# Chang-Tun-Yu/HLS-final-Visual-Odometry

Measured on AMD Instinct MI355X. Metric: stereo frame-pairs/sec (detect+match), KITTI 1241x376; matches bit-exact, higher is better.
Workload: dtype u8; 1 GPU; KITTI 1241x376 stereo quad-match (prev/curr x L/R), default 50x50 bins; noise=0, gpu_max_hw_queues=4, streams_per_gpu=256, frames_in_hbm=8, parallelism=1x independent stream groups

## Files before the change

hls-final-visual-odometry_amd/csrc/kernels_match.hip:

```cpp
#include "vh_dev.h"
#include <algorithm>
#include <cstdlib>
#include <type_traits>

#ifdef VH_FLOW_STATS
__device__ unsigned long long g_flow_stats[12];
extern "C" int32_t vh_debug_flow_stats(unsigned long long *out, int32_t reset) {
  if (hipMemcpyFromSymbol(out, HIP_SYMBOL(g_flow_stats), sizeof(g_flow_stats)) != hipSuccess) return -3;
  if (reset) { unsigned long long z[12] = {0}; if (hipMemcpyToSymbol(HIP_SYMBOL(g_flow_stats), z, sizeof(z)) != hipSuccess) return -3; }
  return 0;
}
#define VH_STAT(k, n) do { if ((threadIdx.x & 63) == 0) atomicAdd(&g_flow_stats[k], (unsigned long long)(n)); } while (0)
#else
#define VH_STAT(k, n) do { } while (0)
#endif

#ifndef VH_MATCH_WAVES
#define VH_MATCH_WAVES 7
#endif
#ifndef VH_SNAKE
#define VH_SNAKE 1
#endif

namespace {

__device__ __forceinline__ int32_t indexed_count(const VhSets &s, int32_t set) { return s.bin_start[(int64_t)set * (s.nbins + 1) + s.nbins]; }

__device__ __forceinline__ int32_t wave_min(int32_t v) {
#pragma unroll
  for (int32_t d = 32; d >= 1; d >>= 1) v = min(v, __shfl_xor(v, d));
  return v;
}
__device__ __forceinline__ int32_t wave_max(int32_t v) {
#pragma unroll
  for (int32_t d = 32; d >= 1; d >>= 1) v = max(v, __shfl_xor(v, d));
  return v;
}

typedef unsigned short us2 __attribute__((ext_vector_type(2)));
__device__ __forceinline__ us2 as_us2(uint32_t x) { return __builtin_bit_cast(us2, x); }
__device__ __forceinline__ uint32_t as_u32(us2 x) { return __builtin_bit_cast(uint32_t, x); }

__device__ __forceinline__ uint32_t sad4(uint32_t a, uint32_t b, uint32_t acc) {
  return __builtin_amdgcn_sad_u8(a, b, acc);
}
__device__ __forceinline__ uint32_t sad4hi(uint32_t a, uint32_t b, uint32_t acc) {
  return __builtin_amdgcn_sad_hi_u8(a, b, acc);
}

template <bool MAX>
__device__ __forceinline__ int32_t row16_allreduce(int32_t v) {
#define VH_ROW_STEP(CTRL)                                                                   \
  {                                                                                         \
    const int32_t t = __builtin_amdgcn_update_dpp(v, v, CTRL, 0xF, 0xF, false);             \
    v = MAX ? max(v, t) : min(v, t);                                                        \
  }
  VH_ROW_STEP(0x128)
  VH_ROW_STEP(0x124)
  VH_ROW_STEP(0x122)
  VH_ROW_STEP(0x121)
#undef VH_ROW_STEP
  return v;
}

template <bool TESTED, bool NEED_UV, class Consume>
__device__ __forceinline__ void walk_region(const VhSets &s, const int32_t *__restrict__ cbs, const uint32_t *__restrict__ cuv,
                                            const uint4 *__restrict__ cdesc, int32_t c, int32_t UB0, int32_t UB1, int32_t VB0,
                                            int32_t VB1, int32_t ULO_MAX, int32_t UHI_MIN, int32_t VA0, int32_t VA1,
                                            Consume consume) {
  const int32_t lane = threadIdx.x & 63;
  const bool merged = !TESTED && VB0 == 0 && VB1 == s.vbn - 1;
  const int32_t UB1w = merged ? UB0 : UB1;
  for (int32_t cb = UB0; cb <= UB1w; cb += 64) {
    const int32_t ncb = min(64, UB1w - cb + 1);
    int32_t t_p0 = 0, t_p1 = 0, t_a0 = 0, t_a1 = 0;
    if (lane < ncb) {
      const int32_t row = (c * s.ubn + cb + lane) * s.vbn;
      t_p0 = cbs[row + VB0]; t_p1 = merged ? cbs[(c * s.ubn + UB1 + 1) * s.vbn] : cbs[row + VB1 + 1];
      if (TESTED) {
        const int32_t ubx = cb + lane;
        const bool in_ = ubx * s.binsize >= ULO_MAX && ubx * s.binsize + s.binsize - 1 <= UHI_MIN;
        t_a0 = in_ ? ((VA0 <= VA1) ? cbs[row + VA0] : t_p1) : 1;
        t_a1 = in_ ? ((VA0 <= VA1) ? cbs[row + VA1 + 1] : t_p1) : 0;
      }
    }
    int32_t ci = -1, pc = -64, p1 = 0;
    const auto advance = [&]() -> bool {
      pc += 64;
      while (pc >= p1) {
        if (++ci >= ncb) return false;
        pc = __builtin_amdgcn_readlane(t_p0, ci); p1 = __builtin_amdgcn_readlane(t_p1, ci);
      }
      return true;
    };
    if (!advance()) continue;
    int32_t pl = min(pc + lane, p1 - 1);
    uint32_t gu = 0;
    if (NEED_UV) gu = cuv[pl];
    uint4 g0 = cdesc[2 * (int64_t)pl], g1 = cdesc[2 * (int64_t)pl + 1];
    for (;;) {
      const int32_t c_pc = pc, c_p1 = p1, c_ci = ci, c_pl = pl;
      const uint32_t c_gu = gu;
      const uint4 c_g0 = g0, c_g1 = g1;
      const bool more = advance();
      if (more) {
        pl = min(pc + lane, p1 - 1);
        if (NEED_UV) gu = cuv[pl];
        g0 = cdesc[2 * (int64_t)pl]; g1 = cdesc[2 * (int64_t)pl + 1];
      }
      int32_t pa0 = 1, pa1 = 0;
      if (TESTED) { pa0 = __builtin_amdgcn_readlane(t_a0, c_ci); pa1 = __builtin_amdgcn_readlane(t_a1, c_ci); }
      consume(c_pc, c_p1, pa0, pa1, c_pl, c_gu, c_g0, c_g1);
      if (!more) break;
    }
  }
}

__device__ __forceinline__ void glds16(const void *gsrc, uint32_t lds_dst) {
  asm volatile("s_mov_b32 m0, %1\n\ts_nop 0\n\tglobal_load_lds_dwordx4 %0, off" ::"v"(gsrc), "s"(lds_dst) : "memory");
}
__device__ __forceinline__ void glds4(const void *gsrc, uint32_t lds_dst) {
  asm volatile("s_mov_b32 m0, %1\n\ts_nop 0\n\tglobal_load_lds_dword %0, off" ::"v"(gsrc), "s"(lds_dst) : "memory");
}
__device__ __forceinline__ uint32_t lds_addr(const void *p) {
  return __builtin_amdgcn_readfirstlane((uint32_t)(uintptr_t)(const __attribute__((address_space(3))) void *)p);
}

template <bool TESTED, class Consume>
__device__ __forceinline__ void walk_region_lds(const VhSets &s, const int32_t *__restrict__ cbs, const uint32_t *__restrict__ cuv,
                                                const uint4 *__restrict__ cdesc, int32_t c, int32_t UB0, int32_t UB1, int32_t VB0,
                                                int32_t VB1, int32_t ULO_MAX, int32_t UHI_MIN, int32_t VA0, int32_t VA1,
                                                uint4 *wD, uint32_t *wU, Consume consume) {
  const int32_t lane = threadIdx.x & 63;
  const uint32_t ldsD = lds_addr(wD), ldsU = lds_addr(wU);
  const bool merged = !TESTED && VB0 == 0 && VB1 == s.vbn - 1;
  const int32_t UB1w = merged ? UB0 : UB1;
  for (int32_t cb = UB0; cb <= UB1w; cb += 64) {
    const int32_t ncb = min(64, UB1w - cb + 1);
    int32_t t_p0 = 0, t_p1 = 0, t_a0 = 0, t_a1 = 0;
    if (lane < ncb) {
      const int32_t row = (c * s.ubn + cb + lane) * s.vbn;
      t_p0 = cbs[row + VB0]; t_p1 = merged ? cbs[(c * s.ubn + UB1 + 1) * s.vbn] : cbs[row + VB1 + 1];
      if (TESTED) {
        const int32_t ubx = cb + lane;
        const bool in_ = ubx * s.binsize >= ULO_MAX && ubx * s.binsize + s.binsize - 1 <= UHI_MIN;
        t_a0 = in_ ? ((VA0 <= VA1) ? cbs[row + VA0] : t_p1) : 1;
        t_a1 = in_ ? ((VA0 <= VA1) ? cbs[row + VA1 + 1] : t_p1) : 0;
      }
    }
    int32_t ci = -1, pc = -64, p1 = 0;
    const auto advance = [&]() -> bool {
      pc += 64;
      while (pc >= p1) {
        if (++ci >= ncb) return false;
        pc = __builtin_amdgcn_readlane(t_p0, ci); p1 = __builtin_amdgcn_readlane(t_p1, ci);
      }
      return true;
    };
    const auto issue = [&](int32_t b) {
      const int32_t pl = min(pc + lane, p1 - 1);
      const uint4 *g = cdesc + 2 * (int64_t)pl;
      glds16(g, ldsD + (uint32_t)b * 2048u); glds16(g + 1, ldsD + (uint32_t)b * 2048u + 1024u);
      if (TESTED) glds4(cuv + pl, ldsU + (uint32_t)b * 256u);
    };
    if (!advance()) continue;
    asm volatile("s_waitcnt lgkmcnt(0)" ::: "memory");
    int32_t buf = 0;
    issue(0);
    for (;;) {
      const int32_t c_pc = pc, c_p1 = p1, c_ci = ci, c_buf = buf;
      const bool more = advance();
      if (more) {
        buf ^= 1;
        asm volatile("s_waitcnt lgkmcnt(0)" ::: "memory");
        issue(buf);
        if (TESTED) asm volatile("s_waitcnt vmcnt(3)" ::: "memory");
        else asm volatile("s_waitcnt vmcnt(2)" ::: "memory");
      } else {
        asm volatile("s_waitcnt vmcnt(0)" ::: "memory");
      }
      int32_t pa0 = 1, pa1 = 0;
      if (TESTED) { pa0 = __builtin_amdgcn_readlane(t_a0, c_ci); pa1 = __builtin_amdgcn_readlane(t_a1, c_ci); }
      consume(c_pc, c_p1, pa0, pa1, (const uint4 *)(wD + c_buf * 128), (const uint32_t *)(wU + c_buf * 64));
      if (!more) break;
    }
  }
}

__device__ __forceinline__ uint64_t tested_key_uniform_query(const uint32_t (&qd)[8], us2 lo2, us2 span2, uint32_t uv2,
                                                             const uint4 &b0, const uint4 &b1, uint32_t relpos) {
  const us2 t = as_us2(uv2) - lo2;
  const us2 m = __builtin_elementwise_min(t, span2);
  uint32_t sad = sad4(qd[0], b0.x, 0);
  sad = sad4(qd[1], b0.y, sad); sad = sad4(qd[2], b0.z, sad); sad = sad4(qd[3], b0.w, sad);
  sad = sad4(qd[4], b1.x, sad); sad = sad4(qd[5], b1.y, sad); sad = sad4(qd[6], b1.z, sad); sad = sad4(qd[7], b1.w, sad);
  return as_u32(t) != as_u32(m) ? ~0ull : (((uint64_t)sad << 32) | relpos);
}
__device__ __forceinline__ uint64_t shfl_xor_u64(uint64_t k, int32_t d) {
  const uint32_t lo = (uint32_t)__shfl_xor((int32_t)(uint32_t)k, d), hi = (uint32_t)__shfl_xor((int32_t)(uint32_t)(k >> 32), d);
  return ((uint64_t)hi << 32) | lo;
}
__device__ __forceinline__ uint64_t wave_min_u64(uint64_t k) {
#pragma unroll
  for (int32_t d = 32; d >= 1; d >>= 1) k = min(k, shfl_xor_u64(k, d));
  return k;
}

enum { KEY_HI16 = 0, KEY_W19 = 1, KEY_64 = 2 };
template <int KM> struct KeyT { typedef uint32_t type; };
template <> struct KeyT<KEY_64> { typedef uint64_t type; };
template <int KM>
__device__ __forceinline__ typename KeyT<KM>::type sad_key(const uint4 &a0, const uint4 &a1, const uint4 &b0, const uint4 &b1, uint32_t seed) {
  if (KM == KEY_HI16) {
    uint32_t key = sad4hi(a0.x, b0.x, seed);
    key = sad4hi(a0.y, b0.y, key); key = sad4hi(a0.z, b0.z, key); key = sad4hi(a0.w, b0.w, key);
    key = sad4hi(a1.x, b1.x, key); key = sad4hi(a1.y, b1.y, key); key = sad4hi(a1.z, b1.z, key); key = sad4hi(a1.w, b1.w, key);
    return (typename KeyT<KM>::type)key;
  }
  uint32_t sad = sad4(a0.x, b0.x, 0);
  sad = sad4(a0.y, b0.y, sad); sad = sad4(a0.z, b0.z, sad); sad = sad4(a0.w, b0.w, sad);
  sad = sad4(a1.x, b1.x, sad); sad = sad4(a1.y, b1.y, sad); sad = sad4(a1.z, b1.z, sad); sad = sad4(a1.w, b1.w, sad);
  if (KM == KEY_W19) return (typename KeyT<KM>::type)((sad << 19) | seed);
  return (typename KeyT<KM>::type)(((uint64_t)sad << 32) | seed);
}
template <int KM>
__device__ __forceinline__ uint64_t key_to_64(typename KeyT<KM>::type k) {
  if (KM == KEY_64) return (uint64_t)k;
  if ((uint32_t)k == 0xFFFFFFFFu) return ~0ull;
  const uint32_t kk = (uint32_t)k;
  return KM == KEY_HI16 ? (((uint64_t)(kk >> 16) << 32) | (kk & 0xFFFFu)) : (((uint64_t)(kk >> 19) << 32) | (kk & 0x7FFFFu));
}
__device__ __forceinline__ int32_t key_mode_of(int32_t class_count, int32_t wide_keys) {
  if (class_count + 64 <= 0x10000 && !wide_keys) return KEY_HI16;
  return class_count <= VH_CLASS_POS_MAX && wide_keys < 2 ? KEY_W19 : KEY_64;
}

#ifndef VH_REDO_G
#define VH_REDO_G 2
#endif
struct RedoGroup {
  uint32_t qd[VH_REDO_G][8];
  us2 lo2[VH_REDO_G];
  int32_t lane[VH_REDO_G], qi[VH_REDO_G], n;
  int32_t umin, umax, vmin, vmax;
};
template <int Q>
__device__ __forceinline__ bool redo_take(uint64_t (&todo)[Q], const uint4 (&a0)[Q], const uint4 (&a1)[Q], const uint32_t (&uv1)[Q],
                                          int32_t radius, int32_t rv, RedoGroup &g) {
  g.n = 0; g.umin = g.vmin = 0x7FFFFFFF; g.umax = g.vmax = -1;
#pragma unroll
  for (int32_t k = 0; k < VH_REDO_G; k++) {
    int32_t fl = -1, fq = 0;
#pragma unroll
    for (int32_t qi = 0; qi < Q; qi++)
      if (fl < 0 && todo[qi]) { fl = (int32_t)__builtin_ctzll(todo[qi]); fq = qi; todo[qi] &= todo[qi] - 1; }
    if (fl < 0) break;
    uint4 x0 = a0[0], x1 = a1[0];
    uint32_t xu = uv1[0];
#pragma unroll
    for (int32_t qi = 1; qi < Q; qi++) if (fq == qi) { x0 = a0[qi]; x1 = a1[qi]; xu = uv1[qi]; }
    g.qd[k][0] = __builtin_amdgcn_readlane(x0.x, fl); g.qd[k][1] = __builtin_amdgcn_readlane(x0.y, fl);
    g.qd[k][2] = __builtin_amdgcn_readlane(x0.z, fl); g.qd[k][3] = __builtin_amdgcn_readlane(x0.w, fl);
    g.qd[k][4] = __builtin_amdgcn_readlane(x1.x, fl); g.qd[k][5] = __builtin_amdgcn_readlane(x1.y, fl);
    g.qd[k][6] = __builtin_amdgcn_readlane(x1.z, fl); g.qd[k][7] = __builtin_amdgcn_readlane(x1.w, fl);
    const uint32_t quv1 = __builtin_amdgcn_readlane(xu, fl);
    const int32_t u1 = (int32_t)(quv1 & 0xFFFF), v1 = (int32_t)(quv1 >> 16);
    g.lo2[k] = us2{(unsigned short)(u1 - radius), (unsigned short)(v1 - rv)};
    g.lane[k] = fl; g.qi[k] = fq; g.n = k + 1;
    g.umin = min(g.umin, u1); g.umax = max(g.umax, u1); g.vmin = min(g.vmin, v1); g.vmax = max(g.vmax, v1);
  }
  return g.n > 0;
}

template <int Q> struct TileOut {
  uint64_t k[Q];
  uint4 a0[Q], a1[Q];
  uint32_t uv1[Q];
  int32_t qpos[Q];
  bool valid[Q];
};

template <int Q, int P, bool SPEC, bool FLOW>
__device__ __forceinline__ void finish_tile(const VhSets &s, const VhMatchArgs &a, int32_t pass, int32_t stream, int32_t qset, int32_t cset,
                                            int32_t c, int32_t pbase, int32_t pcnt, const TileOut<Q> &o,
                                            int32_t *__restrict__ best, int32_t *__restrict__ redo_count) {
  constexpr int L = 64 / P;
  const int32_t lane = threadIdx.x & 63, ph = lane / L;
  const uint32_t *__restrict__ cuv = s.s_uv + (int64_t)cset * s.cap;
  const uint4 *__restrict__ cdesc = (const uint4 *)(s.s_desc + (int64_t)cset * s.cap * 8);
  const int32_t *__restrict__ cbs = s.bin_start + (int64_t)cset * (s.nbins + 1);
  const int32_t rv = FLOW ? a.radius : a.disp_tol;
  const us2 span2 = {(unsigned short)(2 * a.radius), (unsigned short)(2 * rv)};
  const int32_t *__restrict__ cidx = s.s_idx + (int64_t)cset * s.cap;
  const int32_t *__restrict__ qidx = s.s_idx + (int64_t)qset * s.cap;
  int32_t *__restrict__ tbl = best + ((int64_t)stream * 4 + a.pass[pass].slot) * s.cap;
  int32_t res[Q];
  uint64_t todo[Q];
#pragma unroll
  for (int32_t qi = 0; qi < Q; qi++) {
    res[qi] = -1;
    bool fail = false;
    if (o.valid[qi] && ph == 0 && o.k[qi] != ~0ull) {
      int32_t wp = (int32_t)(uint32_t)o.k[qi];
      VH_CHECK_RANGE(s, 7, wp, 0, pcnt);
      res[qi] = pbase + wp;
      if (SPEC) {
        const int32_t u1 = o.uv1[qi] & 0xFFFF, v1 = o.uv1[qi] >> 16;
        const us2 lo2 = {(unsigned short)(u1 - a.radius), (unsigned short)(v1 - rv)};
        const us2 t = as_us2(cuv[res[qi]]) - lo2;
        const us2 m = __builtin_elementwise_min(t, span2);
        fail = as_u32(t) != as_u32(m);
      }
    }
    todo[qi] = SPEC ? __ballot(fail) : 0ull;
  }
  if (SPEC) {
    int32_t nfail = 0;
#pragma unroll
    for (int32_t qi = 0; qi < Q; qi++) nfail += (int32_t)__popcll(todo[qi]);
    if (nfail) {
      VH_STAT(FLOW ? 7 : 10, nfail);
      if (lane == 0) atomicAdd(redo_count, nfail);
      RedoGroup g;
      while (redo_take<Q>(todo, o.a0, o.a1, o.uv1, a.radius, rv, g)) {
        uint64_t kk[VH_REDO_G];
#pragma unroll
        for (int32_t k = 0; k < VH_REDO_G; k++) kk[k] = ~0ull;
        if (FLOW) {
          const auto bin_of = [&](int32_t x, int32_t nb) -> int32_t {
            const uint32_t xx = (uint32_t)max(x, 0);
            return min((int32_t)(s.binsize == 1 ? xx : __umulhi(xx, s.inv_binsize)), nb - 1);
          };
          walk_region<false, true>(s, cbs, cuv, cdesc, c, bin_of(g.umin - a.radius, s.ubn), bin_of(g.umax + a.radius, s.ubn),
                                   bin_of(g.vmin - rv, s.vbn), bin_of(g.vmax + rv, s.vbn), 0, 0, 0, 0,
            [&](int32_t, int32_t, int32_t, int32_t, int32_t pl, uint32_t gu, const uint4 &g0, const uint4 &g1) {
#pragma unroll
              for (int32_t k = 0; k < VH_REDO_G; k++)
                if (k < g.n) kk[k] = min(kk[k], tested_key_uniform_query(g.qd[k], g.lo2[k], span2, gu, g0, g1, (uint32_t)(pl - pbase)));
            });
        } else {
          const int32_t *__restrict__ crs = s.row_start + (int64_t)cset * (4 * s.H + 1);
          const int32_t *__restrict__ cpos = s.r_pos + (int64_t)cset * s.cap;
          const int32_t x0 = __builtin_amdgcn_readfirstlane(crs[c * s.H + max(g.vmin - rv, 0)]);
          const int32_t x1 = __builtin_amdgcn_readfirstlane(crs[c * s.H + min(g.vmax + rv, s.H - 1) + 1]);
          for (int32_t x = x0 + lane; x < x1; x += 64) {
            int32_t cp = cpos[x];
            VH_CHECK_RANGE(s, 3, cp, pbase, pbase + pcnt);
            const uint32_t gu = cuv[cp];
            const uint4 g0 = cdesc[2 * (int64_t)cp], g1 = cdesc[2 * (int64_t)cp + 1];
#pragma unroll
            for (int32_t k = 0; k < VH_REDO_G; k++)
              if (k < g.n) kk[k] = min(kk[k], tested_key_uniform_query(g.qd[k], g.lo2[k], span2, gu, g0, g1, (uint32_t)(cp - pbase)));
          }
        }
#pragma unroll
        for (int32_t k = 0; k < VH_REDO_G; k++)
          if (k < g.n) {
            const uint64_t kf = wave_min_u64(kk[k]);
            int32_t wp = (int32_t)(uint32_t)kf;
            if (kf != ~0ull) VH_CHECK_RANGE(s, 7, wp, 0, pcnt);
            const int32_t r = kf == ~0ull ? -1 : pbase + wp;
#pragma unroll
            for (int32_t qi = 0; qi < Q; qi++) if (lane == g.lane[k] && g.qi[k] == qi) res[qi] = r;
          }
      }
    }
  }
#pragma unroll
  for (int32_t qi = 0; qi < Q; qi++)
    if (o.valid[qi] && ph == 0)
      tbl[qidx[o.qpos[qi]]] = res[qi] < 0 ? 0 : cidx[res[qi]];
}

template <int Q, int P, int KM, bool SPEC>
__device__ __forceinline__ void flow_tile(const VhSets &s, const VhMatchArgs &a, int32_t pass, int32_t stream,
                                          int32_t qset, int32_t cset, int32_t q0, int32_t q1, int32_t c, int32_t col0,
                                          int32_t pbase, int32_t pcnt, uint4 *wD, uint32_t *wU, TileOut<Q> &out) {
  constexpr int L = 64 / P;
  static_assert(L == 8 || L == 16, "every 16-lane row must hold the whole tile (row-wise window reduction)");
  constexpr int TRIP = 2 * P;
  const int32_t lane = threadIdx.x & 63, ph = lane / L, l = lane % L;
  const uint32_t *__restrict__ quv = s.s_uv + (int64_t)qset * s.cap;
  const uint4 *__restrict__ qdesc = (const uint4 *)(s.s_desc + (int64_t)qset * s.cap * 8);
  const uint32_t *__restrict__ cuv = s.s_uv + (int64_t)cset * s.cap;
  const uint4 *__restrict__ cdesc = (const uint4 *)(s.s_desc + (int64_t)cset * s.cap * 8);
  const int32_t *__restrict__ cbs = s.bin_start + (int64_t)cset * (s.nbins + 1);
  const int32_t rv = a.pass[pass].flow ? a.radius : a.disp_tol;

  bool valid[Q];
  uint4 a0[Q], a1[Q];
  uint32_t uv1[Q];
  int32_t v_lo[Q];
  us2 lo2[Q];
  typedef typename KeyT<KM>::type key_t;
  const key_t KNONE = (key_t)~(key_t)0;
  key_t best_key[Q];
  int32_t umin = 0x7FFFFFFF, umax = -1, vmin = 0x7FFFFFFF, vmax = -1;
  int32_t qp[Q];
#pragma unroll
  for (int32_t qi = 0; qi < Q; qi++) {
    const int32_t q = q0 + L * qi + l;
    valid[qi] = q < q1;
    qp[qi] = valid[qi] ? q : q0;
  }
  {
    const int32_t *__restrict__ qbs = s.bin_start + (int64_t)qset * (s.nbins + 1);
    int32_t colb = col0, j = 0;
    int32_t csv = qbs[(c * s.ubn + min(colb + lane, s.ubn)) * s.vbn];
    int32_t A = __builtin_amdgcn_readlane(csv, 0);
    int32_t k[Q];
#pragma unroll
    for (int32_t qi = 0; qi < Q; qi++) k[qi] = qp[qi];
    for (;;) {
      const int32_t B = __builtin_amdgcn_readlane(csv, j + 1);
      if (VH_SNAKE && ((colb + j) & 1)) {
#pragma unroll
        for (int32_t qi = 0; qi < Q; qi++) if (k[qi] >= A && k[qi] < B) qp[qi] = A + B - 1 - k[qi];
      }
      if (B >= q1 || colb + j + 1 >= s.ubn) break;
      A = B;
      if (++j == 63) { colb += 63; j = 0; csv = qbs[(c * s.ubn + min(colb + lane, s.ubn)) * s.vbn]; }
    }
  }
#pragma unroll
  for (int32_t qi = 0; qi < Q; qi++) {
    const int32_t ql = qp[qi];
    uv1[qi] = quv[ql];
    a0[qi] = qdesc[2 * (int64_t)ql]; a1[qi] = qdesc[2 * (int64_t)ql + 1];
    const int32_t u1 = uv1[qi] & 0xFFFF, v1 = uv1[qi] >> 16;
    v_lo[qi] = v1 - rv;
    lo2[qi] = us2{(unsigned short)(u1 - a.radius), (unsigned short)v_lo[qi]};
    best_key[qi] = KNONE;
    umin = min(umin, u1); umax = max(umax, u1); vmin = min(vmin, v1); vmax = max(vmax, v1);
  }
  umin = __builtin_amdgcn_readfirstlane(row16_allreduce<false>(umin));
  umax = __builtin_amdgcn_readfirstlane(row16_allreduce<true>(umax));
  vmin = __builtin_amdgcn_readfirstlane(row16_allreduce<false>(vmin));
  vmax = __builtin_amdgcn_readfirstlane(row16_allreduce<true>(vmax));
  const auto bin_of = [&](int32_t x, int32_t nb) -> int32_t {
    const uint32_t xx = (uint32_t)max(x, 0);
    return min((int32_t)(s.binsize == 1 ? xx : __umulhi(xx, s.inv_binsize)), nb - 1);
  };
  const int32_t UB0 = bin_of(umin - a.radius, s.ubn), UB1 = bin_of(umax + a.radius, s.ubn);
  const int32_t VB0 = bin_of(vmin - rv, s.vbn), VB1 = bin_of(vmax + rv, s.vbn);
  const us2 span2 = {(unsigned short)(2 * a.radius), (unsigned short)(2 * rv)};
  const int32_t ULO_MAX = umax - a.radius, UHI_MIN = umin + a.radius;
  const int32_t VLO_MAX = vmax - rv, VHI_MIN = vmin + rv;
  const int32_t VA0 = SPEC ? 0 : max(VB0, (max(VLO_MAX, 0) + s.binsize - 1) / s.binsize);
  const int32_t VA1 = SPEC ? 0 : min(VB1, (VHI_MIN + 1) / s.binsize - 1);

  auto make_key = [&](auto test, int32_t qi, uint32_t uv2, const uint4 &b0, const uint4 &b1, uint32_t seed) -> key_t {
    constexpr int TEST = decltype(test)::value;
    bool out = false;
    if (TEST == 2) {
      const us2 t = as_us2(uv2) - lo2[qi];
      const us2 m = __builtin_elementwise_min(t, span2);
      out = as_u32(t) != as_u32(m);
    } else if (TEST == 1) {
      out = (uint32_t)((int32_t)(uv2 >> 16) - v_lo[qi]) > (uint32_t)(2 * rv);
    }
    const key_t key = sad_key<KM>(a0[qi], a1[qi], b0, b1, seed);
    return (TEST != 0 && out) ? KNONE : key;
  };
  VH_STAT(0, 1); VH_STAT(5, q1 - q0); VH_STAT(6, UB1 - UB0 + 1);
  walk_region_lds<!SPEC>(s, cbs, cuv, cdesc, c, UB0, UB1, VB0, VB1, ULO_MAX, UHI_MIN, VA0, VA1, wD, wU,
    [&](int32_t pc, int32_t p1, int32_t pa0, int32_t pa1, const uint4 *cD, const uint32_t *cU) {
      VH_STAT(1, 1);
      const int32_t mcnt = min(64, p1 - pc);
      const int32_t jend = (mcnt + TRIP - 1) & ~(TRIP - 1);
      const uint4 *rd = cD + ph;
      const uint32_t *ru = cU + ph;
      uint32_t seedA = (uint32_t)(pc - pbase + ph), seedB = seedA + P;
      int32_t j = 0;
      auto trip = [&](auto test, int32_t o) {
        const uint4 dA0 = rd[o], dA1 = rd[o + 64], dB0 = rd[o + P], dB1 = rd[o + 64 + P];
        uint32_t uA = 0, uB = 0;
        if (decltype(test)::value != 0) { uA = ru[o]; uB = ru[o + P]; }
#pragma unroll
        for (int32_t qi = 0; qi < Q; qi++) {
          const key_t kA = make_key(test, qi, uA, dA0, dA1, seedA + (uint32_t)o), kB = make_key(test, qi, uB, dB0, dB1, seedB + (uint32_t)o);
          best_key[qi] = min(min(kA, kB), best_key[qi]);
        }
      };
      auto run = [&](auto test, int32_t jstop) {
        if (jstop > j) VH_STAT(2 + decltype(test)::value, (jstop - j) / TRIP);
        for (; j + 2 * TRIP <= jstop; j += 2 * TRIP) {
          trip(test, 0); trip(test, TRIP);
          rd += 2 * TRIP; ru += 2 * TRIP; seedA += 2 * TRIP; seedB += 2 * TRIP;
        }
        if (j < jstop) {
          trip(test, 0);
          j += TRIP; rd += TRIP; ru += TRIP; seedA += TRIP; seedB += TRIP;
        }
      };
      if (SPEC) {
        run(std::integral_constant<int, 0>{}, jend);
      } else if (pa0 <= pa1) {
        const int32_t ja = min((min(max(pa0 - pc, 0), mcnt) + TRIP - 1) & ~(TRIP - 1), jend);
        const int32_t jb = max(min(max(pa1 - pc, 0), mcnt) & ~(TRIP - 1), ja);
        run(std::integral_constant<int, 1>{}, ja);
        run(std::integral_constant<int, 0>{}, jb);
        run(std::integral_constant<int, 1>{}, jend);
      } else {
        run(std::integral_constant<int, 2>{}, jend);
      }
    });
#pragma unroll
  for (int32_t qi = 0; qi < Q; qi++) {
    uint64_t k = key_to_64<KM>(best_key[qi]);
#pragma unroll
    for (int32_t d = L; d < 64; d <<= 1) k = min(k, shfl_xor_u64(k, d));
    out.k[qi] = k; out.a0[qi] = a0[qi]; out.a1[qi] = a1[qi]; out.uv1[qi] = uv1[qi]; out.valid[qi] = valid[qi];
    out.qpos[qi] = qp[qi];
  }
}

template <bool SPEC>
__device__ __forceinline__ void flow_pass(const VhSets &s, const VhMatchArgs &a, int32_t pass, int32_t stream, int32_t qset,
                                          int32_t cset, uint4 *wD, uint32_t *wU, int32_t *__restrict__ best, int32_t *__restrict__ redo_count) {
  const int32_t ntile = s.tile_cnt[qset];
  for (int32_t tile = __builtin_amdgcn_readfirstlane(blockIdx.x * 4 + (threadIdx.x >> 6)); tile < ntile;
       tile += gridDim.x * 4) {
    const int4 t = s.tiles[(int64_t)qset * s.max_tiles + tile];
    const int32_t q0 = __builtin_amdgcn_readfirstlane(t.x), q1 = __builtin_amdgcn_readfirstlane(t.y);
    const int32_t c = __builtin_amdgcn_readfirstlane(t.z), col0 = __builtin_amdgcn_readfirstlane(t.w);
    const int32_t *cbs = s.bin_start + (int64_t)cset * (s.nbins + 1);
    const int32_t pbase = __builtin_amdgcn_readfirstlane(cbs[c * s.ubn * s.vbn]);
    const int32_t pend = __builtin_amdgcn_readfirstlane(cbs[(c + 1) * s.ubn * s.vbn]);
    const int32_t km = key_mode_of(pend - pbase, a.wide_keys);
    TileOut<VH_FLOW_Q> out;
    if (km == KEY_HI16) flow_tile<VH_FLOW_Q, VH_FLOW_P, KEY_HI16, SPEC>(s, a, pass, stream, qset, cset, q0, q1, c, col0, pbase, pend - pbase, wD, wU, out);
    else if (km == KEY_W19) flow_tile<VH_FLOW_Q, VH_FLOW_P, KEY_W19, SPEC>(s, a, pass, stream, qset, cset, q0, q1, c, col0, pbase, pend - pbase, wD, wU, out);
    else flow_tile<VH_FLOW_Q, VH_FLOW_P, KEY_64, SPEC>(s, a, pass, stream, qset, cset, q0, q1, c, col0, pbase, pend - pbase, wD, wU, out);
    finish_tile<VH_FLOW_Q, VH_FLOW_P, SPEC, true>(s, a, pass, stream, qset, cset, c, pbase, pend - pbase, out, best, redo_count);
  }
}

template <int Q, int P, int KM, bool SPEC>
__device__ __forceinline__ void rows_tile(const VhSets &s, const VhMatchArgs &a, int32_t pass, int32_t stream, int32_t qset,
                                          int32_t cset, int32_t q0, int32_t q1, int32_t c, int32_t pbase, int32_t pcnt, uint4 *wD,
                                          uint32_t *wU, uint32_t *wV, TileOut<Q> &out) {
  constexpr int L = 64 / P;
  static_assert(L == 8 || L == 16, "every 16-lane row must hold the whole tile");
  constexpr int TRIP = 2 * P;
  const int32_t lane = threadIdx.x & 63, ph = lane / L, l = lane % L;
  const int32_t nrow = 4 * s.H;
  const int32_t *__restrict__ crs = s.row_start + (int64_t)cset * (nrow + 1);
  const int32_t *__restrict__ qpos = s.r_pos + (int64_t)qset * s.cap;
  const uint32_t *__restrict__ quv = s.s_uv + (int64_t)qset * s.cap;
  const uint4 *__restrict__ qdesc = (const uint4 *)(s.s_desc + (int64_t)qset * s.cap * 8);
  const int32_t *__restrict__ cpos = s.r_pos + (int64_t)cset * s.cap;
  const uint32_t *__restrict__ cuv = s.s_uv + (int64_t)cset * s.cap;
  const uint4 *__restrict__ cdesc = (const uint4 *)(s.s_desc + (int64_t)cset * s.cap * 8);

  bool valid[Q];
  uint4 a0[Q], a1[Q];
  uint32_t uv1[Q];
  int32_t qp[Q];
  typedef typename KeyT<KM>::type key_t;
  key_t best_key[Q];
  us2 lo2[Q];
  const us2 span2 = {(unsigned short)(2 * a.radius), (unsigned short)(2 * a.disp_tol)};
  int32_t vmin = 0x7FFFFFFF, vmax = -1;
#pragma unroll
  for (int32_t qi = 0; qi < Q; qi++) {
    const int32_t q = q0 + L * qi + l;
    valid[qi] = q < q1;
    qp[qi] = qpos[valid[qi] ? q : q0];
    VH_CHECK_RANGE(s, 1, qp[qi], 0, s.cap);
    uv1[qi] = quv[qp[qi]];
    a0[qi] = qdesc[2 * (int64_t)qp[qi]]; a1[qi] = qdesc[2 * (int64_t)qp[qi] + 1];
    const int32_t u1 = uv1[qi] & 0xFFFF, v1 = uv1[qi] >> 16;
    lo2[qi] = us2{(unsigned short)(u1 - a.radius), (unsigned short)(v1 - a.disp_tol)};
    best_key[qi] = (key_t)~(key_t)0;
    vmin = min(vmin, v1); vmax = max(vmax, v1);
  }
  vmin = __builtin_amdgcn_readfirstlane(row16_allreduce<false>(vmin));
  vmax = __builtin_amdgcn_readfirstlane(row16_allreduce<true>(vmax));
  VH_STAT(8, 1); VH_STAT(11, q1 - q0);
  const int32_t VLO = max(vmin - a.disp_tol, 0), VHI = min(vmax + a.disp_tol, s.H - 1);
  const int32_t r0 = __builtin_amdgcn_readfirstlane(crs[c * s.H + VLO]);
  const int32_t r1 = __builtin_amdgcn_readfirstlane(crs[c * s.H + VHI + 1]);
  for (int32_t rc = r0; rc < r1; rc += 64) {
    const int32_t mcnt = min(64, r1 - rc);
    int32_t cp = cpos[min(rc + lane, r1 - 1)];
    VH_CHECK_RANGE(s, 2, cp, pbase, pbase + pcnt);
    const uint4 g0 = cdesc[2 * (int64_t)cp], g1 = cdesc[2 * (int64_t)cp + 1];
    uint32_t gu = 0;
    if (!SPEC) gu = cuv[cp];
    asm volatile("s_waitcnt lgkmcnt(0)" ::: "memory");
    wD[lane] = g0; wD[64 + lane] = g1; wU[lane] = (uint32_t)(cp - pbase);
    if (!SPEC) wV[lane] = gu;
    asm volatile("s_waitcnt lgkmcnt(0)" ::: "memory");
    const int32_t jend = (mcnt + TRIP - 1) & ~(TRIP - 1);
    VH_STAT(9, jend / TRIP);
    const uint4 *rd = wD + ph;
    const uint32_t *ru = wU + ph, *rv = wV + ph;
    for (int32_t j = 0; j < jend; j += TRIP) {
      const uint4 dA0 = rd[0], dA1 = rd[64], dB0 = rd[P], dB1 = rd[64 + P];
      const uint32_t sA = ru[0], sB = ru[P];
      uint32_t uA = 0, uB = 0;
      if (!SPEC) { uA = rv[0]; uB = rv[P]; }
#pragma unroll
      for (int32_t qi = 0; qi < Q; qi++) {
        key_t kA = sad_key<KM>(a0[qi], a1[qi], dA0, dA1, sA), kB = sad_key<KM>(a0[qi], a1[qi], dB0, dB1, sB);
        if (!SPEC) {
          const us2 tA = as_us2(uA) - lo2[qi], tB = as_us2(uB) - lo2[qi];
          kA = as_u32(tA) != as_u32(__builtin_elementwise_min(tA, span2)) ? (key_t)~(key_t)0 : kA;
          kB = as_u32(tB) != as_u32(__builtin_elementwise_min(tB, span2)) ? (key_t)~(key_t)0 : kB;
        }
        best_key[qi] = min(min(kA, kB), best_key[qi]);
      }
      rd += TRIP; ru += TRIP; rv += TRIP;
    }
  }
#pragma unroll
  for (int32_t qi = 0; qi < Q; qi++) {
    uint64_t k = key_to_64<KM>(best_key[qi]);
#pragma unroll
    for (int32_t d = L; d < 64; d <<= 1) k = min(k, shfl_xor_u64(k, d));
    out.k[qi] = k; out.a0[qi] = a0[qi]; out.a1[qi] = a1[qi]; out.uv1[qi] = uv1[qi]; out.valid[qi] = valid[qi];
    out.qpos[qi] = qp[qi];
  }
}

template <bool SPEC>
__device__ __forceinline__ void rows_pass(const VhSets &s, const VhMatchArgs &a, int32_t pass, int32_t stream, int32_t qset,
                                          int32_t cset, uint4 *wD, uint32_t *wU, uint32_t *wV, int32_t *__restrict__ best, int32_t *__restrict__ redo_count) {
  const int32_t nrow = 4 * s.H;
  const int32_t *__restrict__ qrs = s.row_start + (int64_t)qset * (nrow + 1);
  int32_t cls_q0[5];
#pragma unroll
  for (int32_t c = 0; c <= 4; c++) cls_q0[c] = __builtin_amdgcn_readfirstlane(qrs[c * s.H]);
  constexpr int T = VH_TILE_Q;
  for (int32_t tile = __builtin_amdgcn_readfirstlane(blockIdx.x * 4 + (threadIdx.x >> 6));; tile += gridDim.x * 4) {
    int32_t c = -1, q0 = 0, q1 = 0, t = tile;
#pragma unroll
    for (int32_t k = 0; k < 4; k++) {
      const int32_t nt = (cls_q0[k + 1] - cls_q0[k] + T - 1) / T;
      if (c < 0 && t < nt) { c = k; q0 = cls_q0[k] + T * t; q1 = min(cls_q0[k + 1], q0 + T); }
      if (c < 0) t -= nt;
    }
    if (c < 0) break;
    const int32_t *cbs = s.bin_start + (int64_t)cset * (s.nbins + 1);
    const int32_t pbase = __builtin_amdgcn_readfirstlane(cbs[c * s.ubn * s.vbn]);
    const int32_t pend = __builtin_amdgcn_readfirstlane(cbs[(c + 1) * s.ubn * s.vbn]);
    const int32_t km = key_mode_of(pend - pbase, a.wide_keys);
    TileOut<VH_FLOW_Q> out;
    if (km == KEY_HI16) rows_tile<VH_FLOW_Q, VH_FLOW_P, KEY_HI16, SPEC>(s, a, pass, stream, qset, cset, q0, q1, c, pbase, pend - pbase, wD, wU, wV, out);
    else if (km == KEY_W19) rows_tile<VH_FLOW_Q, VH_FLOW_P, KEY_W19, SPEC>(s, a, pass, stream, qset, cset, q0, q1, c, pbase, pend - pbase, wD, wU, wV, out);
    else rows_tile<VH_FLOW_Q, VH_FLOW_P, KEY_64, SPEC>(s, a, pass, stream, qset, cset, q0, q1, c, pbase, pend - pbase, wD, wU, wV, out);
    finish_tile<VH_FLOW_Q, VH_FLOW_P, SPEC, false>(s, a, pass, stream, qset, cset, c, pbase, pend - pbase, out, best, redo_count);
  }
}

template <bool SPEC>
__global__ void __launch_bounds__(256) __attribute__((amdgpu_waves_per_eu(VH_MATCH_WAVES, 8)))
match_kernel(VhSets s, VhMatchArgs a, int32_t *__restrict__ best, int32_t *__restrict__ redo) {
  __shared__ uint4 sDesc[4 * 256];
  __shared__ uint32_t sAux[4 * 128];
  __shared__ uint32_t sAux2[SPEC ? 1 : 4 * 64];
  const int32_t pass = blockIdx.y, stream = blockIdx.z;
  if (a.prior && pass == 1) return;
#ifdef VH_EXP_SKIP
  if (VH_EXP_SKIP & (a.pass[pass].flow ? 2 : 1)) return;
#endif
  const int32_t qset = vh_row_set(a, stream, a.pass[pass].qset);
  const int32_t cset = vh_row_set(a, stream, a.pass[pass].cset);
  uint4 *wD = sDesc + (threadIdx.x >> 6) * 256;
  uint32_t *wU = sAux + (threadIdx.x >> 6) * 128;
  uint32_t *wV = sAux2 + (SPEC ? 0 : (threadIdx.x >> 6) * 64);
  int32_t *redo_count = redo + stream;
  if (a.pass[pass].flow) flow_pass<SPEC>(s, a, pass, stream, qset, cset, wD, wU, best, redo_count);
  else rows_pass<SPEC>(s, a, pass, stream, qset, cset, wD, wU, wV, best, redo_count);
}

__global__ void match_prior_kernel(VhSets s, VhMatchArgs a, double u_, double v_, int32_t *__restrict__ best) {
  const int32_t qset = vh_row_set(a, 0, a.pass[0].qset);
  const int32_t cset = vh_row_set(a, 0, a.pass[0].cset);
  const int32_t nq = indexed_count(s, qset);
  const int32_t i = blockIdx.x * blockDim.x + threadIdx.x;
  if (i >= nq) return;
  const int32_t *q = s.feat + ((int64_t)qset * s.cap + i) * 12;
  const int32_t u1 = q[0], v1 = q[1], c = q[3];
  const uint4 a0 = *(const uint4 *)(q + 4), a1 = *(const uint4 *)(q + 8);
  const int32_t rv = a.pass[0].flow ? a.radius : a.disp_tol;
  const int32_t u_lo = u1 - a.radius, u_hi = u1 + a.radius, v_lo = v1 - rv, v_hi = v1 + rv;
  const int32_t ub0 = min(max(u_lo, 0) / s.binsize, s.ubn - 1), ub1 = min(max(u_hi, 0) / s.binsize, s.ubn - 1);
  const int32_t vb0 = min(max(v_lo, 0) / s.binsize, s.vbn - 1), vb1 = min(max(v_hi, 0) / s.binsize, s.vbn - 1);
  const int32_t *__restrict__ cbs = s.bin_start + (int64_t)cset * (s.nbins + 1);
  const uint32_t *__restrict__ cuv = s.s_uv + (int64_t)cset * s.cap;
  const uint4 *__restrict__ cdesc = (const uint4 *)(s.s_desc + (int64_t)cset * s.cap * 8);
  double min_cost = 10000000;
  int32_t min_pos = -1;
  for (int32_t ub = ub0; ub <= ub1; ub++) {
    const int32_t row = (c * s.ubn + ub) * s.vbn;
    for (int32_t p = cbs[row + vb0]; p < cbs[row + vb1 + 1]; p++) {
      const uint32_t uv2 = cuv[p];
      const int32_t u2 = uv2 & 0xFFFF, v2 = uv2 >> 16;
// ... 227 lines not shown
```

Before: 113,900 pairs/s.

## Use scalar-base/offset addressing and permlane-based phase join in match kernel

Replaces 64-bit per-lane pointer arithmetic with 32-bit byte offsets from a uniform base (SGPR base plus VGPR offset for global and global-to-LDS loads). Uniform loads go through the constant address space so they become scalar loads. The cross-phase min-reduction is rewritten with permlane32/permlane16 swaps on 32-bit keys instead of 64-bit shuffles. finish_tile is restructured so each lane owns one query slot, which simplifies the redo bookkeeping. The aim is fewer VALU address instructions, fewer VGPRs and cheaper reductions. The trade-off is that it assumes offsets fit in 32 bits and hard-codes Q=2, P=4.

```diff
diff --git a/hls-final-visual-odometry_amd/csrc/kernels_match.hip b/hls-final-visual-odometry_amd/csrc/kernels_match.hip
--- a/hls-final-visual-odometry_amd/csrc/kernels_match.hip
+++ b/hls-final-visual-odometry_amd/csrc/kernels_match.hip
@@ -62,6 +62,14 @@
 #undef VH_ROW_STEP
   return v;
 }
+
+template <class T>
+__device__ __forceinline__ T ld_off(const T *base, uint32_t byte_off) { return *(const T *)((const char *)base + byte_off); }
+template <class T>
+__device__ __forceinline__ void st_off(T *base, uint32_t byte_off, T x) { *(T *)((char *)base + byte_off) = x; }
+template <class T>
+__device__ __forceinline__ T ld_uniform(const T *p) { return *(const __attribute__((address_space(4))) T *)(uintptr_t)p; }
+__device__ __forceinline__ int32_t ld_uniform_i32(const int32_t *p) { return __builtin_amdgcn_readfirstlane(ld_uniform(p)); }
 
 template <bool TESTED, bool NEED_UV, class Consume>
 __device__ __forceinline__ void walk_region(const VhSets &s, const int32_t *__restrict__ cbs, const uint32_t *__restrict__ cuv,
@@ -76,7 +84,8 @@
     int32_t t_p0 = 0, t_p1 = 0, t_a0 = 0, t_a1 = 0;
     if (lane < ncb) {
       const int32_t row = (c * s.ubn + cb + lane) * s.vbn;
-      t_p0 = cbs[row + VB0]; t_p1 = merged ? cbs[(c * s.ubn + UB1 + 1) * s.vbn] : cbs[row + VB1 + 1];
+      t_p0 = ld_off(cbs, (uint32_t)(row + VB0) * 4u);
+      t_p1 = ld_off(cbs, (uint32_t)(merged ? (c * s.ubn + UB1 + 1) * s.vbn : row + VB1 + 1) * 4u);
       if (TESTED) {
         const int32_t ubx = cb + lane;
         const bool in_ = ubx * s.binsize >= ULO_MAX && ubx * s.binsize + s.binsize - 1 <= UHI_MIN;
@@ -116,11 +125,11 @@
   }
 }
 
-__device__ __forceinline__ void glds16(const void *gsrc, uint32_t lds_dst) {
-  asm volatile("s_mov_b32 m0, %1\n\ts_nop 0\n\tglobal_load_lds_dwordx4 %0, off" ::"v"(gsrc), "s"(lds_dst) : "memory");
-}
-__device__ __forceinline__ void glds4(const void *gsrc, uint32_t lds_dst) {
-  asm volatile("s_mov_b32 m0, %1\n\ts_nop 0\n\tglobal_load_lds_dword %0, off" ::"v"(gsrc), "s"(lds_dst) : "memory");
+__device__ __forceinline__ void glds16(const void *gbase, uint32_t byte_off, uint32_t lds_dst) {
+  asm volatile("s_mov_b32 m0, %2\n\ts_nop 0\n\tglobal_load_lds_dwordx4 %0, %1" ::"v"(byte_off), "s"(gbase), "s"(lds_dst) : "memory");
+}
+__device__ __forceinline__ void glds4(const void *gbase, uint32_t byte_off, uint32_t lds_dst) {
+  asm volatile("s_mov_b32 m0, %2\n\ts_nop 0\n\tglobal_load_lds_dword %0, %1" ::"v"(byte_off), "s"(gbase), "s"(lds_dst) : "memory");
 }
 __device__ __forceinline__ uint32_t lds_addr(const void *p) {
   return __builtin_amdgcn_readfirstlane((uint32_t)(uintptr_t)(const __attribute__((address_space(3))) void *)p);
@@ -133,6 +142,7 @@
                                                 uint4 *wD, uint32_t *wU, Consume consume) {
   const int32_t lane = threadIdx.x & 63;
   const uint32_t ldsD = lds_addr(wD), ldsU = lds_addr(wU);
+  const uint32_t lane32 = (uint32_t)lane * 32u;
   const bool merged = !TESTED && VB0 == 0 && VB1 == s.vbn - 1;
   const int32_t UB1w = merged ? UB0 : UB1;
   for (int32_t cb = UB0; cb <= UB1w; cb += 64) {
@@ -140,7 +150,8 @@
     int32_t t_p0 = 0, t_p1 = 0, t_a0 = 0, t_a1 = 0;
     if (lane < ncb) {
       const int32_t row = (c * s.ubn + cb + lane) * s.vbn;
-      t_p0 = cbs[row + VB0]; t_p1 = merged ? cbs[(c * s.ubn + UB1 + 1) * s.vbn] : cbs[row + VB1 + 1];
+      t_p0 = ld_off(cbs, (uint32_t)(row + VB0) * 4u);
+      t_p1 = ld_off(cbs, (uint32_t)(merged ? (c * s.ubn + UB1 + 1) * s.vbn : row + VB1 + 1) * 4u);
       if (TESTED) {
         const int32_t ubx = cb + lane;
         const bool in_ = ubx * s.binsize >= ULO_MAX && ubx * s.binsize + s.binsize - 1 <= UHI_MIN;
@@ -158,10 +169,9 @@
       return true;
     };
     const auto issue = [&](int32_t b) {
-      const int32_t pl = min(pc + lane, p1 - 1);
-      const uint4 *g = cdesc + 2 * (int64_t)pl;
-      glds16(g, ldsD + (uint32_t)b * 2048u); glds16(g + 1, ldsD + (uint32_t)b * 2048u + 1024u);
-      if (TESTED) glds4(cuv + pl, ldsU + (uint32_t)b * 256u);
+      const uint32_t off = min((uint32_t)pc * 32u + lane32, (uint32_t)(p1 - 1) * 32u);
+      glds16(cdesc, off, ldsD + (uint32_t)b * 2048u); glds16(cdesc, off + 16u, ldsD + (uint32_t)b * 2048u + 1024u);
+      if (TESTED) glds4(cuv, off >> 3, ldsU + (uint32_t)b * 256u);
     };
     if (!advance()) continue;
     asm volatile("s_waitcnt lgkmcnt(0)" ::: "memory");
@@ -223,16 +233,30 @@
   if (KM == KEY_W19) return (typename KeyT<KM>::type)((sad << 19) | seed);
   return (typename KeyT<KM>::type)(((uint64_t)sad << 32) | seed);
 }
-template <int KM>
-__device__ __forceinline__ uint64_t key_to_64(typename KeyT<KM>::type k) {
-  if (KM == KEY_64) return (uint64_t)k;
-  if ((uint32_t)k == 0xFFFFFFFFu) return ~0ull;
-  const uint32_t kk = (uint32_t)k;
-  return KM == KEY_HI16 ? (((uint64_t)(kk >> 16) << 32) | (kk & 0xFFFFu)) : (((uint64_t)(kk >> 19) << 32) | (kk & 0x7FFFFu));
-}
 __device__ __forceinline__ int32_t key_mode_of(int32_t class_count, int32_t wide_keys) {
   if (class_count + 64 <= 0x10000 && !wide_keys) return KEY_HI16;
   return class_count <= VH_CLASS_POS_MAX && wide_keys < 2 ? KEY_W19 : KEY_64;
+}
+
+template <int Q, int P, int KM>
+__device__ __forceinline__ int32_t join_phases(const typename KeyT<KM>::type (&best_key)[Q]) {
+  static_assert(Q == 2 && P == 4, "the join splits the wave into two slots of two 16-lane rows");
+  if (KM == KEY_64) {
+    uint64_t k[Q];
+#pragma unroll
+    for (int32_t qi = 0; qi < Q; qi++) {
+      k[qi] = (uint64_t)best_key[qi];
+#pragma unroll
+      for (int32_t d = 16; d < 64; d <<= 1) k[qi] = min(k[qi], shfl_xor_u64(k[qi], d));
+    }
+    const uint64_t kk = (threadIdx.x & 32) ? k[1] : k[0];
+    return kk == ~0ull ? -1 : (int32_t)(uint32_t)kk;
+  }
+  const auto h = __builtin_amdgcn_permlane32_swap((uint32_t)best_key[0], (uint32_t)best_key[1], false, false);
+  const uint32_t kh = min(h[0], h[1]);
+  const auto r = __builtin_amdgcn_permlane16_swap(kh, kh, false, false);
+  const uint32_t k = min(r[0], r[1]);
+  return k == 0xFFFFFFFFu ? -1 : (int32_t)(k & (KM == KEY_HI16 ? 0xFFFFu : 0x7FFFFu));
 }
 
 #ifndef VH_REDO_G
@@ -241,20 +265,18 @@
 struct RedoGroup {
   uint32_t qd[VH_REDO_G][8];
   us2 lo2[VH_REDO_G];
-  int32_t lane[VH_REDO_G], qi[VH_REDO_G], n;
+  int32_t lane[VH_REDO_G], n;
   int32_t umin, umax, vmin, vmax;
 };
 template <int Q>
-__device__ __forceinline__ bool redo_take(uint64_t (&todo)[Q], const uint4 (&a0)[Q], const uint4 (&a1)[Q], const uint32_t (&uv1)[Q],
+__device__ __forceinline__ bool redo_take(uint64_t &todo, const uint4 (&a0)[Q], const uint4 (&a1)[Q], const uint32_t (&uv1)[Q],
                                           int32_t radius, int32_t rv, RedoGroup &g) {
   g.n = 0; g.umin = g.vmin = 0x7FFFFFFF; g.umax = g.vmax = -1;
 #pragma unroll
   for (int32_t k = 0; k < VH_REDO_G; k++) {
-    int32_t fl = -1, fq = 0;
-#pragma unroll
-    for (int32_t qi = 0; qi < Q; qi++)
-      if (fl < 0 && todo[qi]) { fl = (int32_t)__builtin_ctzll(todo[qi]); fq = qi; todo[qi] &= todo[qi] - 1; }
-    if (fl < 0) break;
+    if (!todo) break;
+    const int32_t fl = (int32_t)__builtin_ctzll(todo), fq = fl >> 5;
+    todo &= todo - 1;
     uint4 x0 = a0[0], x1 = a1[0];
     uint32_t xu = uv1[0];
 #pragma unroll
@@ -266,14 +288,14 @@
     const uint32_t quv1 = __builtin_amdgcn_readlane(xu, fl);
     const int32_t u1 = (int32_t)(quv1 & 0xFFFF), v1 = (int32_t)(quv1 >> 16);
     g.lo2[k] = us2{(unsigned short)(u1 - radius), (unsigned short)(v1 - rv)};
-    g.lane[k] = fl; g.qi[k] = fq; g.n = k + 1;
+    g.lane[k] = fl; g.n = k + 1;
     g.umin = min(g.umin, u1); g.umax = max(g.umax, u1); g.vmin = min(g.vmin, v1); g.vmax = max(g.vmax, v1);
   }
   return g.n > 0;
 }
 
 template <int Q> struct TileOut {
-  uint64_t k[Q];
+  int32_t wp;
   uint4 a0[Q], a1[Q];
   uint32_t uv1[Q];
   int32_t qpos[Q];
@@ -284,8 +306,8 @@
 __device__ __forceinline__ void finish_tile(const VhSets &s, const VhMatchArgs &a, int32_t pass, int32_t stream, int32_t qset, int32_t cset,
                                             int32_t c, int32_t pbase, int32_t pcnt, const TileOut<Q> &o,
                                             int32_t *__restrict__ best, int32_t *__restrict__ redo_count) {
-  constexpr int L = 64 / P;
-  const int32_t lane = threadIdx.x & 63, ph = lane / L;
+  static_assert(Q == 2 && P == 4, "one query per lane: slot lane >> 5, on the first 16-lane row of each half (join_phases)");
+  const int32_t lane = threadIdx.x & 63;
   const uint32_t *__restrict__ cuv = s.s_uv + (int64_t)cset * s.cap;
   const uint4 *__restrict__ cdesc = (const uint4 *)(s.s_desc + (int64_t)cset * s.cap * 8);
   const int32_t *__restrict__ cbs = s.bin_start + (int64_t)cset * (s.nbins + 1);
@@ -294,31 +316,27 @@
   const int32_t *__restrict__ cidx = s.s_idx + (int64_t)cset * s.cap;
   const int32_t *__restrict__ qidx = s.s_idx + (int64_t)qset * s.cap;
   int32_t *__restrict__ tbl = best + ((int64_t)stream * 4 + a.pass[pass].slot) * s.cap;
-  int32_t res[Q];
-  uint64_t todo[Q];
-#pragma unroll
-  for (int32_t qi = 0; qi < Q; qi++) {
-    res[qi] = -1;
-    bool fail = false;
-    if (o.valid[qi] && ph == 0 && o.k[qi] != ~0ull) {
-      int32_t wp = (int32_t)(uint32_t)o.k[qi];
-      VH_CHECK_RANGE(s, 7, wp, 0, pcnt);
-      res[qi] = pbase + wp;
-      if (SPEC) {
-        const int32_t u1 = o.uv1[qi] & 0xFFFF, v1 = o.uv1[qi] >> 16;
-        const us2 lo2 = {(unsigned short)(u1 - a.radius), (unsigned short)(v1 - rv)};
-        const us2 t = as_us2(cuv[res[qi]]) - lo2;
-        const us2 m = __builtin_elementwise_min(t, span2);
-        fail = as_u32(t) != as_u32(m);
-      }
-    }
-    todo[qi] = SPEC ? __ballot(fail) : 0ull;
+  const bool hi = lane & 32;
+  const bool mine = !(lane & 16) && (hi ? o.valid[1] : o.valid[0]);
+  const uint32_t uv1 = hi ? o.uv1[1] : o.uv1[0];
+  const int32_t qpos = hi ? o.qpos[1] : o.qpos[0];
+  int32_t res = -1;
+  bool fail = false;
+  if (mine && o.wp >= 0) {
+    int32_t wp = o.wp;
+    VH_CHECK_RANGE(s, 7, wp, 0, pcnt);
+    res = pbase + wp;
+    if (SPEC) {
+      const us2 lo2 = as_us2(uv1) - us2{(unsigned short)a.radius, (unsigned short)rv};
+      const us2 t = as_us2(ld_off(cuv, (uint32_t)res * 4u)) - lo2;
+      const us2 m = __builtin_elementwise_min(t, span2);
+      fail = as_u32(t) != as_u32(m);
+    }
   }
   if (SPEC) {
-    int32_t nfail = 0;
-#pragma unroll
-    for (int32_t qi = 0; qi < Q; qi++) nfail += (int32_t)__popcll(todo[qi]);
-    if (nfail) {
+    uint64_t todo = __ballot(fail);
+    if (todo) {
+      const int32_t nfail = (int32_t)__popcll(todo);
       VH_STAT(FLOW ? 7 : 10, nfail);
       if (lane == 0) atomicAdd(redo_count, nfail);
       RedoGroup g;
@@ -341,8 +359,8 @@
         } else {
           const int32_t *__restrict__ crs = s.row_start + (int64_t)cset * (4 * s.H + 1);
           const int32_t *__restrict__ cpos = s.r_pos + (int64_t)cset * s.cap;
-          const int32_t x0 = __builtin_amdgcn_readfirstlane(crs[c * s.H + max(g.vmin - rv, 0)]);
-          const int32_t x1 = __builtin_amdgcn_readfirstlane(crs[c * s.H + min(g.vmax + rv, s.H - 1) + 1]);
+          const int32_t x0 = ld_uniform_i32(crs + c * s.H + max(g.vmin - rv, 0));
+          const int32_t x1 = ld_uniform_i32(crs + c * s.H + min(g.vmax + rv, s.H - 1) + 1);
           for (int32_t x = x0 + lane; x < x1; x += 64) {
             int32_t cp = cpos[x];
             VH_CHECK_RANGE(s, 3, cp, pbase, pbase + pcnt);
@@ -359,17 +377,12 @@
             const uint64_t kf = wave_min_u64(kk[k]);
             int32_t wp = (int32_t)(uint32_t)kf;
             if (kf != ~0ull) VH_CHECK_RANGE(s, 7, wp, 0, pcnt);
-            const int32_t r = kf == ~0ull ? -1 : pbase + wp;
-#pragma unroll
-            for (int32_t qi = 0; qi < Q; qi++) if (lane == g.lane[k] && g.qi[k] == qi) res[qi] = r;
+            if (lane == g.lane[k]) res = kf == ~0ull ? -1 : pbase + wp;
           }
       }
     }
   }
-#pragma unroll
-  for (int32_t qi = 0; qi < Q; qi++)
-    if (o.valid[qi] && ph == 0)
-      tbl[qidx[o.qpos[qi]]] = res[qi] < 0 ? 0 : cidx[res[qi]];
+  if (mine) st_off(tbl, (uint32_t)ld_off(qidx, (uint32_t)qpos * 4u) * 4u, res < 0 ? 0 : ld_off(cidx, (uint32_t)res * 4u));
 }
 
 template <int Q, int P, int KM, bool SPEC>
@@ -406,7 +419,7 @@
   {
     const int32_t *__restrict__ qbs = s.bin_start + (int64_t)qset * (s.nbins + 1);
     int32_t colb = col0, j = 0;
-    int32_t csv = qbs[(c * s.ubn + min(colb + lane, s.ubn)) * s.vbn];
+    int32_t csv = ld_off(qbs, (uint32_t)((c * s.ubn + min(colb + lane, s.ubn)) * s.vbn) * 4u);
     int32_t A = __builtin_amdgcn_readlane(csv, 0);
     int32_t k[Q];
 #pragma unroll
@@ -419,14 +432,14 @@
       }
       if (B >= q1 || colb + j + 1 >= s.ubn) break;
       A = B;
-      if (++j == 63) { colb += 63; j = 0; csv = qbs[(c * s.ubn + min(colb + lane, s.ubn)) * s.vbn]; }
+      if (++j == 63) { colb += 63; j = 0; csv = ld_off(qbs, (uint32_t)((c * s.ubn + min(colb + lane, s.ubn)) * s.vbn) * 4u); }
     }
   }
 #pragma unroll
   for (int32_t qi = 0; qi < Q; qi++) {
     const int32_t ql = qp[qi];
-    uv1[qi] = quv[ql];
-    a0[qi] = qdesc[2 * (int64_t)ql]; a1[qi] = qdesc[2 * (int64_t)ql + 1];
+    uv1[qi] = ld_off(quv, (uint32_t)ql * 4u);
+    a0[qi] = ld_off(qdesc, (uint32_t)ql * 32u); a1[qi] = ld_off(qdesc, (uint32_t)ql * 32u + 16u);
     const int32_t u1 = uv1[qi] & 0xFFFF, v1 = uv1[qi] >> 16;
     v_lo[qi] = v1 - rv;
     lo2[qi] = us2{(unsigned short)(u1 - a.radius), (unsigned short)v_lo[qi]};
@@ -505,12 +518,10 @@
         run(std::integral_constant<int, 2>{}, jend);
       }
     });
+  out.wp = join_phases<Q, P, KM>(best_key);
 #pragma unroll
   for (int32_t qi = 0; qi < Q; qi++) {
-    uint64_t k = key_to_64<KM>(best_key[qi]);
-#pragma unroll
-    for (int32_t d = L; d < 64; d <<= 1) k = min(k, shfl_xor_u64(k, d));
-    out.k[qi] = k; out.a0[qi] = a0[qi]; out.a1[qi] = a1[qi]; out.uv1[qi] = uv1[qi]; out.valid[qi] = valid[qi];
+    out.a0[qi] = a0[qi]; out.a1[qi] = a1[qi]; out.uv1[qi] = uv1[qi]; out.valid[qi] = valid[qi];
     out.qpos[qi] = qp[qi];
   }
 }
@@ -518,15 +529,16 @@
 template <bool SPEC>
 __device__ __forceinline__ void flow_pass(const VhSets &s, const VhMatchArgs &a, int32_t pass, int32_t stream, int32_t qset,
                                           int32_t cset, uint4 *wD, uint32_t *wU, int32_t *__restrict__ best, int32_t *__restrict__ redo_count) {
-  const int32_t ntile = s.tile_cnt[qset];
+  const int32_t ntile = ld_uniform_i32(s.tile_cnt + qset);
   for (int32_t tile = __builtin_amdgcn_readfirstlane(blockIdx.x * 4 + (threadIdx.x >> 6)); tile < ntile;
        tile += gridDim.x * 4) {
-    const int4 t = s.tiles[(int64_t)qset * s.max_tiles + tile];
+    typedef int32_t i32x4 __attribute__((ext_vector_type(4)));
+    const i32x4 t = ld_uniform((const i32x4 *)(s.tiles + (int64_t)qset * s.max_tiles + tile));
     const int32_t q0 = __builtin_amdgcn_readfirstlane(t.x), q1 = __builtin_amdgcn_readfirstlane(t.y);
     const int32_t c = __builtin_amdgcn_readfirstlane(t.z), col0 = __builtin_amdgcn_readfirstlane(t.w);
     const int32_t *cbs = s.bin_start + (int64_t)cset * (s.nbins + 1);
-    const int32_t pbase = __builtin_amdgcn_readfirstlane(cbs[c * s.ubn * s.vbn]);
-    const int32_t pend = __builtin_amdgcn_readfirstlane(cbs[(c + 1) * s.ubn * s.vbn]);
+    const int32_t pbase = ld_uniform_i32(cbs + c * s.ubn * s.vbn);
+    const int32_t pend = ld_uniform_i32(cbs + (c + 1) * s.ubn * s.vbn);
     const int32_t km = key_mode_of(pend - pbase, a.wide_keys);
     TileOut<VH_FLOW_Q> out;
     if (km == KEY_HI16) flow_tile<VH_FLOW_Q, VH_FLOW_P, KEY_HI16, SPEC>(s, a, pass, stream, qset, cset, q0, q1, c, col0, pbase, pend - pbase, wD, wU, out);
@@ -566,10 +578,10 @@
   for (int32_t qi = 0; qi < Q; qi++) {
     const int32_t q = q0 + L * qi + l;
     valid[qi] = q < q1;
-    qp[qi] = qpos[valid[qi] ? q : q0];
+    qp[qi] = ld_off(qpos, (uint32_t)(valid[qi] ? q : q0) * 4u);
     VH_CHECK_RANGE(s, 1, qp[qi], 0, s.cap);
-    uv1[qi] = quv[qp[qi]];
-    a0[qi] = qdesc[2 * (int64_t)qp[qi]]; a1[qi] = qdesc[2 * (int64_t)qp[qi] + 1];
+    uv1[qi] = ld_off(quv, (uint32_t)qp[qi] * 4u);
+    a0[qi] = ld_off(qdesc, (uint32_t)qp[qi] * 32u); a1[qi] = ld_off(qdesc, (uint32_t)qp[qi] * 32u + 16u);
     const int32_t u1 = uv1[qi] & 0xFFFF, v1 = uv1[qi] >> 16;
     lo2[qi] = us2{(unsigned short)(u1 - a.radius), (unsigned short)(v1 - a.disp_tol)};
     best_key[qi] = (key_t)~(key_t)0;
@@ -579,15 +591,15 @@
   vmax = __builtin_amdgcn_readfirstlane(row16_allreduce<true>(vmax));
   VH_STAT(8, 1); VH_STAT(11, q1 - q0);
   const int32_t VLO = max(vmin - a.disp_tol, 0), VHI = min(vmax + a.disp_tol, s.H - 1);
-  const int32_t r0 = __builtin_amdgcn_readfirstlane(crs[c * s.H + VLO]);
-  const int32_t r1 = __builtin_amdgcn_readfirstlane(crs[c * s.H + VHI + 1]);
+  const int32_t r0 = ld_uniform_i32(crs + c * s.H + VLO);
+  const int32_t r1 = ld_uniform_i32(crs + c * s.H + VHI + 1);
   for (int32_t rc = r0; rc < r1; rc += 64) {
     const int32_t mcnt = min(64, r1 - rc);
-    int32_t cp = cpos[min(rc + lane, r1 - 1)];
+    int32_t cp = ld_off(cpos, (uint32_t)min(rc + lane, r1 - 1) * 4u);
     VH_CHECK_RANGE(s, 2, cp, pbase, pbase + pcnt);
-    const uint4 g0 = cdesc[2 * (int64_t)cp], g1 = cdesc[2 * (int64_t)cp + 1];
+    const uint4 g0 = ld_off(cdesc, (uint32_t)cp * 32u), g1 = ld_off(cdesc, (uint32_t)cp * 32u + 16u);
     uint32_t gu = 0;
-    if (!SPEC) gu = cuv[cp];
+    if (!SPEC) gu = ld_off(cuv, (uint32_t)cp * 4u);
     asm volatile("s_waitcnt lgkmcnt(0)" ::: "memory");
     wD[lane] = g0; wD[64 + lane] = g1; wU[lane] = (uint32_t)(cp - pbase);
     if (!SPEC) wV[lane] = gu;
@@ -614,12 +626,10 @@
       rd += TRIP; ru += TRIP; rv += TRIP;
     }
   }
+  out.wp = join_phases<Q, P, KM>(best_key);
 #pragma unroll
   for (int32_t qi = 0; qi < Q; qi++) {
-    uint64_t k = key_to_64<KM>(best_key[qi]);
-#pragma unroll
-    for (int32_t d = L; d < 64; d <<= 1) k = min(k, shfl_xor_u64(k, d));
-    out.k[qi] = k; out.a0[qi] = a0[qi]; out.a1[qi] = a1[qi]; out.uv1[qi] = uv1[qi]; out.valid[qi] = valid[qi];
+    out.a0[qi] = a0[qi]; out.a1[qi] = a1[qi]; out.uv1[qi] = uv1[qi]; out.valid[qi] = valid[qi];
     out.qpos[qi] = qp[qi];
   }
 }
@@ -631,7 +641,7 @@
   const int32_t *__restrict__ qrs = s.row_start + (int64_t)qset * (nrow + 1);
   int32_t cls_q0[5];
 #pragma unroll
-  for (int32_t c = 0; c <= 4; c++) cls_q0[c] = __builtin_amdgcn_readfirstlane(qrs[c * s.H]);
+  for (int32_t c = 0; c <= 4; c++) cls_q0[c] = ld_uniform_i32(qrs + c * s.H);
   constexpr int T = VH_TILE_Q;
   for (int32_t tile = __builtin_amdgcn_readfirstlane(blockIdx.x * 4 + (threadIdx.x >> 6));; tile += gridDim.x * 4) {
     int32_t c = -1, q0 = 0, q1 = 0, t = tile;
@@ -643,8 +653,8 @@
     }
     if (c < 0) break;
     const int32_t *cbs = s.bin_start + (int64_t)cset * (s.nbins + 1);
-    const int32_t pbase = __builtin_amdgcn_readfirstlane(cbs[c * s.ubn * s.vbn]);
-    const int32_t pend = __builtin_amdgcn_readfirstlane(cbs[(c + 1) * s.ubn * s.vbn]);
+    const int32_t pbase = ld_uniform_i32(cbs + c * s.ubn * s.vbn);
+    const int32_t pend = ld_uniform_i32(cbs + (c + 1) * s.ubn * s.vbn);
     const int32_t km = key_mode_of(pend - pbase, a.wide_keys);
     TileOut<VH_FLOW_Q> out;
     if (km == KEY_HI16) rows_tile<VH_FLOW_Q, VH_FLOW_P, KEY_HI16, SPEC>(s, a, pass, stream, qset, cset, q0, q1, c, pbase, pend - pbase, wD, wU, wV, out);
```

Result: faster. 116,200 pairs/s (median of 6 runs) (+2.0%).
